# Kirkice/3DGaussian

Hardware: AMD Instinct MI355X
Metric: Mpixels/sec fwd+bwd @1M Gaussians 800×800; PSNR vs torch ref (higher is better)
Workload: dtype f32 (splat contractions on v_mfma_f32_32x32x16_f16 with f32 accumulation; every operand in two round-to-nearest f16 pieces, pre-scaled into f16's normal range, three piece products: <= 3*2^-22 per product, forward and backward; no-depth-gradient mode); 1 GPU; C4: 1000000 Gaussians, 50 orbit views 800x800, fwd+bwd+grad all-reduce+Adam per step; gaussians=1000000, views=50, width=800, height=800, tile=32, seed=0, parallelism=view-sharded dp1, gaussian_order=morton (trainer layout, re-established every 16 steps)

## Files before the change

### 3dgaussian_amd/csrc/gr_hip.hip

```cpp

#include <hip/hip_runtime.h>
#include <hipcub/hipcub.hpp>
#include <rocprim/rocprim.hpp>

#include <cmath>
#include <cstdint>
#include <cstdio>
#include <cstdlib>
#include <cstring>
#include <atomic>
#include <mutex>
#include <string>
#include <type_traits>
#include <vector>

#include "../../include/gr_hip.h"

#ifndef GR_TAIL2
#define GR_TAIL2 1
#endif
#ifndef GR_DEBUG_PREP_REPS
#define GR_DEBUG_PREP_REPS 1
#endif
#ifndef GR_DEBUG_BIN_REPS
// ... 324 lines not shown
  int* ticket;
};

struct Scratch {
  uint32_t* keys_in;
  int* ids_in;
  float* fwd_part;
  int2* pairs_in;
  int2* pairs_sorted;
  void* sort_tmp;
};

inline int64_t item_cap(int tiles, int64_t K, int ch = CH) { return (K + ch - 1) / ch + tiles; }
constexpr int UF32_FRAGS = 2 * 4 * 2 * 2 * 64;
constexpr int UF32_STRIDE = UF32_FRAGS + 64;
struct TileCfg {
  int T, ch;
  size_t part_floats, uf_frags;
};
constexpr int UF_FRAGS16 = 2 * 3 * 3 * 64;
static int64_t tune_env(const char* name);
inline int chunk_of(const gr_view* v, int base, int64_t K) {
  static const int64_t force = tune_env("GR_TUNE_CHUNK");
  int64_t c = base;
  if (v->chunk > 0) {
    c = v->chunk;
  } else if (force > 0) {
    c = force;
  } else if (K >= 0) {
    c = 512;
    while (c < base && 2 * c * 1024 <= K) c *= 2;
  }
  return (int)std::min<int64_t>(8192, std::max<int64_t>(64, (c + 63) / 64 * 64));
}
inline TileCfg tile_cfg(const gr_view* v, int64_t K = -1) {
  return tile_of(v) == T32 ? TileCfg{T32, chunk_of(v, CH32, K), (size_t)4 * TP32, (size_t)UF32_STRIDE}
                           : TileCfg{T, chunk_of(v, CH, K), (size_t)5 * TP, (size_t)UF_FRAGS16};
}

constexpr int FAN_STRIDE = 32;
__host__ __device__ inline size_t fan_offset(int tiles) { return ((size_t)tiles + 1 + FAN_STRIDE - 1) / FAN_STRIDE * FAN_STRIDE; }

size_t bins_fixed(int vtiles, int64_t K, size_t off[8], int ch = CH) {
  const int tiles = vtiles;
  const size_t kk = (size_t)(K > 0 ? K : 1);
  const size_t cap = (size_t)item_cap(tiles, K, ch);
  size_t o = 0;
  off[0] = o; o = align_up(o + (short_keys(tiles) ? 1 : kk) * sizeof(uint32_t));
  off[1] = o; o = align_up(o + kk * sizeof(int));
  off[2] = o; o = align_up(o + (size_t)tiles * sizeof(int2));
  off[3] = o; o = align_up(o + cap * sizeof(int4));
  off[4] = o; o = align_up(o + 2 * sizeof(int));
  off[5] = o; o = align_up(o + (size_t)tiles * sizeof(int));
  off[6] = o; o = align_up(o + kk * sizeof(int));
  off[7] = o; o = align_up(o + (fan_offset(tiles / 2) + 9 * FAN_STRIDE) * sizeof(int));
  return o;
}

size_t scratch_fixed(int vtiles, int64_t K, size_t off[5], int ch = CH, size_t part_floats = (size_t)5 * TP) {
  const int tiles = vtiles;
  const size_t kk = (size_t)(K > 0 ? K : 1);
  const size_t cap = (size_t)item_cap(tiles, K, ch);
  size_t o = 0;
  off[0] = o; o = align_up(o + kk * sizeof(uint32_t));
  off[1] = o; o = align_up(o + kk * sizeof(int));
  off[2] = o; o = align_up(o + cap * part_floats * sizeof(float));
  off[3] = o; o = align_up(o + (short_keys(tiles) ? 1 : kk) * sizeof(int2));
  off[4] = o; o = align_up(o + (short_keys(tiles) ? 1 : kk) * sizeof(int2));
  return o;
}


static int64_t tune_env(const char* name) {
  const char* e = std::getenv(name);
  return e ? std::atoll(e) : 0;
}
inline int tsort_waves(int tiles) {
  static const int64_t force = tune_env("GR_TUNE_PLACE_WAVES");
  const int64_t per_wave = 4ll * tiles, budget = 65536 - 512;
  const int w = 4 * per_wave <= budget ? 4 : 2 * per_wave <= budget ? 2 : 1;
  if (force == 8 && 8 * per_wave <= 81920 - 512) return 8;
  return force == 1 || force == 2 || force == 4 ? std::min<int>(w, (int)force) : w;
}

#ifndef GR_TS_SEG
#define GR_TS_SEG 24
#endif
constexpr int TS_SEG = GR_TS_SEG;

inline int col_width(int64_t K, int tiles) {
  static const int64_t force = tune_env("GR_TUNE_COL_TARGET");
  const int waves = tsort_waves(tiles);
  if (force > 0) return (int)((force + 64 * waves - 1) / (64 * waves) * (64 * waves));
  const int64_t kk = K > 0 ? K : 1;
  int64_t pw = 64ll * TS_SEG;
  auto cols_of = [&](int64_t w) { return (kk + w * waves - 1) / (w * waves); };
  while ((int64_t)tiles * cols_of(pw) > (1ll << 28) || ((int64_t)tiles * cols_of(pw) > kk / 2 && cols_of(2 * pw) >= 1024))
    pw *= 2;
  return (int)(pw * waves);
}
inline int cols_of(int64_t Kz, int cw) { return (int)((Kz + cw - 1) / cw); }

size_t tile_sort_tmp_bytes(int n, int64_t K, int tiles) {
  if (short_keys(tiles)) {
    const int st = tiles / 2;
    const size_t cells = (size_t)st * cols_of(K > 0 ? K : 1, col_width(K, st));
    (void)n;
    return 4 * align_up(cells * sizeof(int)) + 2 * align_up((size_t)st * sizeof(int));
  }
  size_t tmp = 0;
  (void)hipcub::DeviceRadixSort::SortPairs(nullptr, tmp, (const uint32_t*)nullptr, (uint32_t*)nullptr, (const int2*)nullptr,
                                           (int2*)nullptr, (int)(K > 0 ? K : 1), 0, bits_for((uint32_t)tiles),
                                           (hipStream_t)0);
  return tmp;
}

template <typename KeyT>
size_t sort_tmp_bytes(int64_t K, int bits) {
  size_t tmp = 0;
  (void)hipcub::DeviceRadixSort::SortPairs(nullptr, tmp, (KeyT*)nullptr, (KeyT*)nullptr, (int*)nullptr, (int*)nullptr,
                                     (int)(K > 0 ? K : 1), 0, bits, (hipStream_t)0);
  return tmp;
}

Bins bins_view(void* base, int tiles, int64_t K, int ch = CH) {
  size_t off[8];
  bins_fixed(tiles, K, off, ch);
  char* b = (char*)base;
  Bins r;
  r.keys = (uint32_t*)(b + off[0]);
  r.pairs = (int*)(b + off[1]);
  r.ranges = (int2*)(b + off[2]);
  r.items = (int4*)(b + off[3]);
  r.num_items = (int*)(b + off[4]);
  r.tile_item0 = (int*)(b + off[5]);
  r.pos_of = (int*)(b + off[6]);
  r.ticket = (int*)(b + off[7]);
  return r;
}

Scratch scratch_view(void* base, int tiles, int64_t K, int ch = CH, size_t part_floats = (size_t)5 * TP) {
  size_t off[5];
  const size_t fixed = scratch_fixed(tiles, K, off, ch, part_floats);
  char* b = (char*)base;
  Scratch r;
  r.keys_in = (uint32_t*)(b + off[0]);
  r.ids_in = (int*)(b + off[1]);
  r.fwd_part = (float*)(b + off[2]);
  r.pairs_in = (int2*)(b + off[3]);
  r.pairs_sorted = (int2*)(b + off[4]);
  r.sort_tmp = b + fixed;
  return r;
}

template <int NW>
__device__ __forceinline__ unsigned long long block_exclusive_scan(unsigned long long x, unsigned long long* sh,
                                                                   unsigned long long& total) {
  const int lane = (int)threadIdx.x & 63, w = (int)threadIdx.x >> 6;
  unsigned long long inc = x;
#pragma unroll
  for (int o = 1; o < 64; o <<= 1) {
    const unsigned long long y = __shfl_up(inc, o);
    if (lane >= o) inc += y;
  }
  __syncthreads();
  if (lane == 63) sh[w] = inc;
// ... 569 lines not shown
  k_tile_count_body(a.Z, a.tiles, b.block, b.grid);
}
__global__ __launch_bounds__(256) void k_tile_count(k_tile_count_args a) {
  k_tile_count_run(a, own_block());
}
__global__ __launch_bounds__(256) void k_tile_count_views(VBatch<k_tile_count_args> B) {
  const VBlock b = vbatch_block(B);
  k_tile_count_run(B.a[b.view], b);
}


#ifndef GR_CS_T
#define GR_CS_T 16
#endif
#ifndef GR_CS_THREADS
#define GR_CS_THREADS 256
#endif
#ifndef GR_CS_R
#define GR_CS_R 96
#endif
constexpr int CS_T = GR_CS_T, CS_G = GR_CS_THREADS / GR_CS_T, CS_R = GR_CS_R;

__device__ __forceinline__ void tile_colscan_block(const TZone& zz, int tiles, int bx) {
  const int cols = zz.cols;
  const int* __restrict__ M = zz.M;
  int* __restrict__ S = zz.S;
  int* __restrict__ T = zz.T;
  __shared__ int part[CS_G][CS_T + 1];
  const int tl = (int)threadIdx.x % CS_T, g = (int)threadIdx.x / CS_T;
  const int t = bx * CS_T + tl;
  const int per = (cols + CS_G - 1) / CS_G;
  const int c0 = min(cols, g * per), c1 = min(cols, c0 + per);
  const bool regs = per <= CS_R;
  int val[CS_R];
  int sum = 0;
  if (t < tiles) {
    if (regs) {
#pragma unroll
      for (int q = 0; q < CS_R; ++q) val[q] = c0 + q < c1 ? M[(size_t)(c0 + q) * tiles + t] : 0;
#pragma unroll
      for (int q = 0; q < CS_R; ++q) sum += val[q];
    } else {
#pragma unroll 8
      for (int c = c0; c < c1; ++c) sum += M[(size_t)c * tiles + t];
    }
  }
  part[g][tl] = sum;
  __syncthreads();
  if (g == 0) {
    int run = 0;
    for (int u = 0; u < CS_G; ++u) {
      const int v = part[u][tl];
      part[u][tl] = run;
      run += v;
    }
    if (t < tiles) st_through(&T[t], run);
  }
  __syncthreads();
  if (t < tiles) {
    int run = part[g][tl];
    if (regs) {
#pragma unroll
      for (int q = 0; q < CS_R; ++q)
        if (c0 + q < c1) {
          S[(size_t)(c0 + q) * tiles + t] = run;
          run += val[q];
        }
    } else {
#pragma unroll 8
      for (int c = c0; c < c1; ++c) {
        const int v = M[(size_t)c * tiles + t];
        S[(size_t)c * tiles + t] = run;
        run += v;
      }
    }
  }
}


template <bool THROUGH, int NT>
__device__ void work_items_zones(int tiles, int Kc, const int* __restrict__ Tc, const int* __restrict__ Tt,
                                 int2* __restrict__ ranges, int4* __restrict__ items, int* __restrict__ num_items,
                                 int* __restrict__ tile_item0, int* __restrict__ ticket, int ch);
__device__ __forceinline__ void k_tile_colscan_body(TZones Z, int tiles, int2* __restrict__ ranges,
                                                             int4* __restrict__ items, int* __restrict__ num_items,
                                                             int* __restrict__ tile_item0, int* __restrict__ ticket, const BI blockIdx, const BI gridDim) {
  __shared__ int last;
  const TZone zz = zone_at(Z, (int)blockIdx.y);
  if (zz.K > 0) tile_colscan_block(zz, tiles, (int)blockIdx.x);
  const int nb = (int)(gridDim.x * gridDim.y);
  if (!arrive_last_of(ticket + fan_offset(tiles), nb, (int)(blockIdx.y * gridDim.x + blockIdx.x), &last)) return;
  const TZone z0 = zone_at(Z, 0), z1 = zone_at(Z, 1);
  work_items_zones<true, GR_CS_THREADS>(tiles, z1.zbase, z0.K > 0 ? z0.T : nullptr, z1.K > 0 ? z1.T : nullptr,
                                  ranges, items, num_items, tile_item0, ticket, Z.ch);
}
struct k_tile_colscan_args {
  TZones Z;
  int tiles;
  int2* ranges;
  int4* items;
  int* num_items;
  int* tile_item0;
  int* ticket;
};
__device__ __forceinline__ void k_tile_colscan_run(const k_tile_colscan_args& a, const VBlock& b) {
  k_tile_colscan_body(a.Z, a.tiles, a.ranges, a.items, a.num_items, a.tile_item0, a.ticket, b.block, b.grid);
}
__global__ __launch_bounds__(GR_CS_THREADS) void k_tile_colscan(k_tile_colscan_args a) {
  k_tile_colscan_run(a, own_block());
}
__global__ __launch_bounds__(GR_CS_THREADS) void k_tile_colscan_views(VBatch<k_tile_colscan_args> B) {
  const VBlock b = vbatch_block(B);
  k_tile_colscan_run(B.a[b.view], b);
}



__device__ __forceinline__ void ts_load(int64_t kb, int64_t k1, int64_t klast, int lane, const uint16_t* __restrict__ keys,
                                        const int* __restrict__ ids_in, int (&d)[TS_SEG], int (&id)[TS_SEG]) {
#pragma unroll
  for (int j = 0; j < TS_SEG; ++j) {
    const int64_t k = kb + j * 64 + lane;
    const int64_t kc = k < k1 ? k : klast;
    const int key = (int)keys[kc];
    id[j] = ids_in[kc];
    d[j] = k < k1 ? key : -1;
  }
}

__device__ __forceinline__ void ts_place(int lane, int bits, int* my, const int (&d)[TS_SEG], const int (&id)[TS_SEG],
                                         int kseg, int* __restrict__ pairs_out, int* __restrict__ pos_of) {
  const uint64_t below = (1ull << lane) - 1ull;
#pragma unroll
  for (int j = 0; j < TS_SEG; ++j) {
    const bool ok = d[j] >= 0;
    const uint64_t live = __ballot(ok);
    if (live == 0) break;
    const int rel = d[j] - __builtin_amdgcn_readfirstlane(d[j]) + TS_RH;
    const bool near = __ballot(ok && (unsigned)rel >= 2u * TS_RH) == 0;
    const int key = near ? rel : d[j];
    const int nb = near && TS_RB < bits ? TS_RB : bits;
    unsigned mlo = (unsigned)live, mhi = (unsigned)(live >> 32);
    for (int b = 0; b < nb; ++b) {
      const int bm = __builtin_amdgcn_sbfe(key, b, 1);
      const uint64_t v = __ballot(bm != 0);
      mlo &= ~((unsigned)v ^ (unsigned)bm);
      mhi &= ~((unsigned)(v >> 32) ^ (unsigned)bm);
    }
    const uint64_t m = ((uint64_t)mhi << 32) | mlo;
    if (ok) {
      const int pos = my[d[j]] + __popcll(m & below);
      pairs_out[pos] = id[j];
      pos_of[kseg + j * 64 + lane] = pos;
      __builtin_amdgcn_wave_barrier();
      if ((m >> lane) == 1ull) my[d[j]] = pos + 1;
    }
  }
}

constexpr int RUNQ = 10;
template <bool THROUGH, int NT>
__device__ void work_items_zones(int tiles, int Kc, const int* __restrict__ Tc, const int* __restrict__ Tt,
                                 int2* __restrict__ ranges, int4* __restrict__ items, int* __restrict__ num_items,
                                 int* __restrict__ tile_item0, int* __restrict__ ticket, int ch) {
  __shared__ unsigned long long sh[NT / 64];
  const int per = (tiles + NT - 1) / NT;
  const int t0 = min(tiles, (int)threadIdx.x * per), t1 = min(tiles, t0 + per);
  int rc_[RUNQ], rt_[RUNQ];
  auto ld = [&](const int* T, int t) { return !T || t >= t1 ? 0 : THROUGH ? ld_through(T + t) : T[t]; };
  auto load_run = [&](int b) {
#pragma unroll
    for (int q = 0; q < RUNQ; ++q) {
      rc_[q] = ld(Tc, b + q);
      rt_[q] = ld(Tt, b + q);
    }
  };
  int sc = 0, st = 0, sch = 0, se = 0;
  for (int b = t0; b < t1; b += RUNQ) {
    load_run(b);
#pragma unroll
    for (int q = 0; q < RUNQ; ++q) {
      const int nc = rc_[q], nt = rt_[q];
      sc += nc;
      st += nt;
      const int nch = chunks_of(nc, ch) + chunks_of(nt, ch);
      sch += nch;
      se += nch == 0 && b + q < t1;
    }
  }
  unsigned long long t1v, t2v;
  const unsigned long long e1 = block_exclusive_scan<NT / 64>((unsigned long long)sc | ((unsigned long long)st << 32), sh, t1v);
  const unsigned long long e2 = block_exclusive_scan<NT / 64>((unsigned long long)sch | ((unsigned long long)se << 32), sh, t2v);
  sc = (int)(e1 & 0xffffffffull);
  st = (int)(e1 >> 32);
  sch = (int)(e2 & 0xffffffffull);
  se = (int)(e2 >> 32);
  const int total = (int)(t2v & 0xffffffffull), empties = (int)(t2v >> 32);
  se += total;
  for (int b = t0; b < t1; b += RUNQ) {
    if (t1 - t0 > RUNQ) load_run(b);
#pragma unroll
    for (int q = 0; q < RUNQ; ++q) {
      const int t = b + q;
      if (t < t1) {
        const int nc = rc_[q], nt = rt_[q];
        const int2 rc = nc > 0 ? make_int2(sc, sc + nc) : make_int2(0, 0);
        const int2 rt = nt > 0 ? make_int2(Kc + st, Kc + st + nt) : make_int2(0, 0);
        const int chc = chunks_of(nc, ch), cht = chunks_of(nt, ch);
        ranges[2 * t] = rc;
        ranges[2 * t + 1] = rt;
        tile_item0[2 * t] = sch;
        tile_item0[2 * t + 1] = sch + chc;
        ticket[t] = 0;
        for (int c = 0; c < chc; ++c) items[sch + c] = make_int4(2 * t, rc.x + c * ch, min(rc.y, rc.x + (c + 1) * ch), c);
        for (int c = 0; c < cht; ++c)
          items[sch + chc + c] = make_int4(2 * t + 1, rt.x + c * ch, min(rt.y, rt.x + (c + 1) * ch), c);
        if (chc + cht == 0) {
          tile_item0[2 * t] = tile_item0[2 * t + 1] = se;
          items[se++] = make_int4(2 * t, 0, 0, 0);
        }
        sc += nc;
        st += nt;
        sch += chc + cht;
      }
    }
  }
  if (threadIdx.x == 0) {
    num_items[0] = total + empties;
    num_items[1] = total;
  }
  if (threadIdx.x < 9) ticket[fan_offset(tiles) + FAN_STRIDE * threadIdx.x] = 0;
}

#ifndef GR_PLACE_WAVES
#define GR_PLACE_WAVES 3
#endif
constexpr int TS_CQ = 8;
template <int WAVES>
__device__ __forceinline__ void k_tile_place_body(TZones Z, int tiles, int bits,
                                                                    const int2* __restrict__ ranges,
                                                                    int* __restrict__ pairs_out, int* __restrict__ pos_of, const BI blockIdx, const BI gridDim) {
  extern __shared__ int cur[];
  constexpr int NT = 64 * WAVES;
  int c;
  const int zone = tzone_of(Z, (int)blockIdx.x, c);
  const TZone zz = zone_at(Z, zone);
  const int64_t K = zz.K;
  const int zbase = zz.zbase;
  const uint16_t* __restrict__ keys = zz.keys;
  const int* __restrict__ ids_in = zz.ids;
  const int* __restrict__ S = zz.S + (size_t)c * tiles;
  const int w = (int)threadIdx.x >> 6, lane = (int)threadIdx.x & 63;
  int* my = cur + (size_t)w * tiles;
  int64_t kc0, kc1;
  column_range(Z, K, c, kc0, kc1);
  if (kc1 <= kc0) return;
  const int64_t steps = (kc1 - kc0 + 63) / 64, wsteps = (steps + WAVES - 1) / WAVES;
  const int64_t k0 = min(kc1, kc0 + (int64_t)w * wsteps * 64), k1 = min(kc1, k0 + wsteps * 64);
  const int nseg = (int)((wsteps + TS_SEG - 1) / TS_SEG);
  int d[TS_SEG], id[TS_SEG];
  ts_load(k0, k1, K - 1, lane, keys, ids_in, d, id);
  int rx[TS_CQ], sx[TS_CQ];
  auto load_bases = [&](int t0) {
#pragma unroll
    for (int q = 0; q < TS_CQ; ++q) {
      const int t = min(t0 + q * NT, tiles - 1);
      rx[q] = ranges[2 * t + zone].x;
      sx[q] = S[t];
    }
  };
  load_bases((int)threadIdx.x);
  for (int t = lane; t < tiles; t += 64) my[t] = 0;
  __builtin_amdgcn_wave_barrier();
  for (int seg = 0; seg < nseg; ++seg) {
    if (seg > 0) ts_load(k0 + (int64_t)seg * 64 * TS_SEG, k1, K - 1, lane, keys, ids_in, d, id);
#pragma unroll
    for (int j = 0; j < TS_SEG; ++j) atomicAdd(&my[d[j] < 0 ? 0 : d[j]], (d[j] < 0 ? 0 : 1) + (id[j] >> 31));
  }
  __syncthreads();
  for (int t0 = threadIdx.x; t0 < tiles; t0 += TS_CQ * NT) {
    if (t0 != (int)threadIdx.x) load_bases(t0);
#pragma unroll
    for (int q = 0; q < TS_CQ; ++q) {
      const int t = t0 + q * NT;
      if (t >= tiles) break;
      int r = rx[q] + sx[q];
#pragma unroll
      for (int u = 0; u < WAVES; ++u) {
        const int m = cur[(size_t)u * tiles + t];
        cur[(size_t)u * tiles + t] = r;
        r += m;
      }
    }
  }
  __syncthreads();
  if (nseg == 1) {
    ts_place(lane, bits, my, d, id, zbase + (int)k0, pairs_out, pos_of);
  } else {
    for (int seg = 0; seg < nseg; ++seg) {
      ts_load(k0 + (int64_t)seg * 64 * TS_SEG, k1, K - 1, lane, keys, ids_in, d, id);
      ts_place(lane, bits, my, d, id, zbase + (int)(k0 + (int64_t)seg * 64 * TS_SEG), pairs_out, pos_of);
    }
  }
}
struct k_tile_place_args {
  TZones Z;
  int tiles;
  int bits;
  const int2* ranges;
  int* pairs_out;
  int* pos_of;
};
template <int WAVES>
__device__ __forceinline__ void k_tile_place_run(const k_tile_place_args& a, const VBlock& b) {
  k_tile_place_body<WAVES>(a.Z, a.tiles, a.bits, a.ranges, a.pairs_out, a.pos_of, b.block, b.grid);
}
template <int WAVES>
__global__ __launch_bounds__(64 * WAVES, GR_PLACE_WAVES) void k_tile_place(k_tile_place_args a) {
  k_tile_place_run<WAVES>(a, own_block());
}
template <int WAVES>
__global__ __launch_bounds__(64 * WAVES, GR_PLACE_WAVES) void k_tile_place_views(VBatch<k_tile_place_args> B) {
  const VBlock b = vbatch_block(B);
  k_tile_place_run<WAVES>(B.a[b.view], b);
}


__device__ __forceinline__ void split3(float x, float& hi, float& mid, float& lo) {
  hi = __uint_as_float(__float_as_uint(x) & 0xffff0000u);
  const float r1 = x - hi;
  mid = __uint_as_float(__float_as_uint(r1) & 0xffff0000u);
  lo = r1 - mid;
}
__device__ __forceinline__ unsigned pack_bf16(float a, float b) {
  return __builtin_amdgcn_perm(__float_as_uint(b), __float_as_uint(a), 0x07060302u);
}

typedef short s16x8 __attribute__((ext_vector_type(8)));
typedef float f32x16 __attribute__((ext_vector_type(16)));

__device__ __forceinline__ s16x8 as_frag(uint4 u) {
  s16x8 f;
  __builtin_memcpy(&f, &u, sizeof(f));
  return f;
}

__device__ __forceinline__ void split3_frag(const float (&v)[8], s16x8 (&f)[3]) {
  float hi[8], mid[8], lo[8];
#pragma unroll
  for (int j = 0; j < 8; ++j) split3(v[j], hi[j], mid[j], lo[j]);
  f[0] = as_frag(make_uint4(pack_bf16(hi[0], hi[1]), pack_bf16(hi[2], hi[3]), pack_bf16(hi[4], hi[5]), pack_bf16(hi[6], hi[7])));
  f[1] = as_frag(make_uint4(pack_bf16(mid[0], mid[1]), pack_bf16(mid[2], mid[3]), pack_bf16(mid[4], mid[5]),
                            pack_bf16(mid[6], mid[7])));
  f[2] = as_frag(make_uint4(pack_bf16(lo[0], lo[1]), pack_bf16(lo[2], lo[3]), pack_bf16(lo[4], lo[5]), pack_bf16(lo[6], lo[7])));
}
typedef __bf16 bf16x2_t __attribute__((ext_vector_type(2)));
typedef float f32x2_t __attribute__((ext_vector_type(2)));
__device__ __forceinline__ void split2_frag(const float (&v)[8], s16x8 (&f)[2]) {
  unsigned h[4], l[4];
#pragma unroll
  for (int p = 0; p < 4; ++p) {
    const f32x2_t x = {v[2 * p], v[2 * p + 1]};
    const bf16x2_t hb = __builtin_convertvector(x, bf16x2_t);
    __builtin_memcpy(&h[p], &hb, 4);
    const f32x2_t r = {x.x - __uint_as_float(h[p] << 16), x.y - __uint_as_float(h[p] & 0xffff0000u)};
    const bf16x2_t lb = __builtin_convertvector(r, bf16x2_t);
    __builtin_memcpy(&l[p], &lb, 4);
  }
  f[0] = as_frag(make_uint4(h[0], h[1], h[2], h[3]));
  f[1] = as_frag(make_uint4(l[0], l[1], l[2], l[3]));
}
__device__ __forceinline__ f32x4 mfma16(const s16x8& a, const s16x8& b, f32x4 c) {
  return __builtin_amdgcn_mfma_f32_16x16x32_bf16(a, b, c, 0, 0, 0);
}
__device__ __forceinline__ f32x4 mfma16_split3(const s16x8 (&a)[3], const s16x8 (&b)[3], f32x4 c) {
  c = mfma16(a[2], b[0], c);
  c = mfma16(a[1], b[1], c);
  c = mfma16(a[0], b[2], c);
  c = mfma16(a[1], b[0], c);
  c = mfma16(a[0], b[1], c);
  return mfma16(a[0], b[0], c);
}
template <bool B3>
__device__ __forceinline__ f32x4 mfma16_split2(const s16x8 (&a)[2], const s16x8 (&b)[3], f32x4 c) {
  c = mfma16(a[1], b[0], c);
  if constexpr (B3) c = mfma16(a[0], b[2], c);
  c = mfma16(a[0], b[1], c);
  return mfma16(a[0], b[0], c);
}

__device__ __forceinline__ void split2_frag2(const f32x2_t (&v)[4], s16x8 (&f)[2]) {
  float u[8];
#pragma unroll
  for (int p = 0; p < 4; ++p) {
    u[2 * p] = v[p].x;
    u[2 * p + 1] = v[p].y;
  }
  split2_frag(u, f);
}

__device__ __forceinline__ void split3_frag2(const f32x2_t (&v)[4], s16x8 (&f)[3]) {
  float u[8];
#pragma unroll
  for (int p = 0; p < 4; ++p) {
    u[2 * p] = v[p].x;
    u[2 * p + 1] = v[p].y;
  }
// ... 3797 lines not shown
  char* q = (char*)c.sc.sort_tmp;
  for (int z = 0; z < 2; ++z) {
    TZone& zz = Z.z[z];
    zz.K = Kr[z];
    zz.cols = cols_of(Kr[z], Z.cw);
    zz.zbase = z == 0 ? 0 : (int)Kc;
    zz.keys = (const uint16_t*)c.sc.keys_in + (z == 0 ? 0 : Kc);
    zz.ids = c.sc.ids_in + (z == 0 ? 0 : Kc);
    zz.M = (int*)q;
    q += align_up(cells * sizeof(int));
    zz.S = (int*)q;
    q += align_up(cells * sizeof(int));
    zz.T = (int*)q;
    q += align_up((size_t)c.tiles * sizeof(int));
  }
  return Z;
}

struct ParamsIn {
  const float *means = nullptr, *scales = nullptr, *colors = nullptr;
  int color_dim = 3;
  const float* opacities = nullptr;
};
struct GradsOut {
  float *d_means = nullptr, *d_scales = nullptr, *d_colors = nullptr, *d_opacities = nullptr;
  int accumulate = 0;
};
struct ViewLoss {
  const float *t_rgb = nullptr, *t_mask = nullptr;
  float w_sil = 0.0f;
  const float* t_depth = nullptr;
  float w_depth = 0.0f, g_scale = 0.0f;
  float* loss_out = nullptr;
  bool ssim_entry = false;
  float w_dssim = 0.0f;
  bool expo_entry = false;
  const float* exposure = nullptr;
  float* d_exposure = nullptr;
  bool wgt_entry = false;
  const float* t_weight = nullptr;
};
struct BwdRequest {
  const gr_view* view = nullptr;
  int n = 0;
  const gr_plan* plan = nullptr;
  const void *geom = nullptr, *bins = nullptr;
  const float* saved = nullptr;
  void* ws = nullptr;
  size_t ws_bytes = 0;
  void* stream = nullptr;
  ParamsIn params;
  const float *g_rgb = nullptr, *g_alpha = nullptr, *g_depth = nullptr;
  ViewLoss loss;
  GradsOut grads;
  float *sums = nullptr, *sums3 = nullptr;
  const int* sum_index = nullptr;
};

static L1Args fit_l1_args(const ViewCtx& c, const ViewLoss& vl) {
  L1Args l1{vl.t_rgb, vl.t_mask, vl.w_sil, vl.g_scale, nullptr};
  if (!vl.t_rgb) return l1;
  l1.tile_loss = c.w.tile_loss;
  l1.loss_out = vl.loss_out;
  l1.n1 = (int64_t)(3 * c.HW);
  l1.n2 = (int64_t)(vl.t_mask ? c.HW : 0);
  if (vl.t_depth) {
    l1.t_depth = vl.t_depth;
    l1.w_depth = vl.w_depth;
    l1.dscal = c.w.dscal;
  }
  return l1;
}

static k_emit_offsets_args emit_offsets_args(const ViewCtx& c) {
  return {c.vk, c.n, (const int4*)c.g.rect, (const Cnt2*)c.g.counts, (const unsigned long long*)c.g.total,
          (Cnt2*)c.g.offsets, (const float4*)c.g.rec, (uint16_t*)c.sc.keys_in, c.sc.ids_in,
          c.b.ticket + fan_offset(c.tiles)};
}
static k_tile_count_args tile_count_args(const ViewCtx& c, const TZones& Z) { return {Z, c.tiles}; }
static k_tile_colscan_args tile_colscan_args(const ViewCtx& c, const TZones& Z) {
  return {Z, c.tiles, c.b.ranges, c.b.items, c.b.num_items, c.b.tile_item0, c.b.ticket};
}
static k_tile_place_args tile_place_args(const ViewCtx& c, const TZones& Z) {
  return {Z, c.tiles, bits_for((uint32_t)c.tiles), (const int2*)c.b.ranges, c.b.pairs, c.b.pos_of};
}
static k_raster_fwd_mfma_args fwd_mfma_args(const ViewCtx& c, float* out_rgb, float* out_alpha, float* out_depth,
                                            float* saved, const L1Args& l1, uint4* UF) {
  return {c.vk, c.n, (const int4*)c.b.items, (const int*)c.b.num_items, (const int2*)c.b.ranges, (const int*)c.b.pairs,
          (const float4*)c.g.rec, c.sc.fwd_part, out_rgb, out_alpha, out_depth, (float4*)saved,
          saved ? saved + 4 * c.HW : nullptr, l1, UF, (const int*)(c.n > 0 && c.K() > 0 ? c.g.f16_sa : nullptr),
          (const int*)c.b.tile_item0, c.b.ticket, c.tc.ch};
}
static k_fwd32_l1_args fwd32_args(const ViewCtx& c, float* out_rgb, float* out_alpha, const L1Args& l1, uint4* UF) {
  return {c.vk, c.n, (const int4*)c.b.items, (const int*)c.b.num_items, (const int2*)c.b.ranges, (const int*)c.b.pairs,
          (const float4*)c.g.rec, c.sc.fwd_part, out_rgb, out_alpha, l1, UF,
          (const int*)(c.n > 0 && c.K() > 0 ? c.g.f16_sa : nullptr), (const int*)c.b.tile_item0, c.b.ticket, c.tc.ch};
}
static k_raster_bwd_bf16_args bwd_bf16_args(const ViewCtx& c, float* depth3) {
  return {c.vk, c.n, (const int4*)c.b.items, (const int*)c.b.num_items, (const int*)c.b.pairs, (const float4*)c.g.rec,
          (const uint4*)c.w.UF, c.w.partials, depth3};
}
static k_bwd32_args bwd32_args(const ViewCtx& c) {
  return {c.vk, c.n, (const int4*)c.b.items, (const int*)c.b.num_items, (const int*)c.b.pairs, (const float4*)c.g.rec,
          (const uint4*)c.w.UF, c.w.partials};
}
static k_depth_tile_max_args depth_tile_max_args(const ViewCtx& c, const float* saved) {
  return {c.vk, (const float4*)saved, saved + 4 * c.HW, c.w.tile_aux, c.w.dscal, c.b.ticket};
}
static k_depth_tile_sums_args depth_tile_sums_args(const ViewCtx& c, const float* saved, const float* t_depth,
                                                   float w_depth, float g_scale) {
  return {c.vk, (const float4*)saved, saved + 4 * c.HW, t_depth, c.w.dscal, c.w.tile_loss, c.w.tile_aux, (int64_t)c.HW,
          w_depth, g_scale, c.b.ticket};
}
static k_pixel_grads_args pixel_grads_args(const ViewCtx& c, const float* saved, const float* g_rgb, const float* g_alpha,
                                           const float* g_depth, int pieces, const L1Args& l1, bool depth) {
  return {c.vk, (const float4*)saved, saved + 4 * c.HW, g_rgb, g_alpha, g_depth, c.w.UF, pieces, l1, depth, c.b.ticket};
}
static k_gather_view_args gather_args(const ViewCtx& c, float* sums, float* sums3, bool depth) {
  return {c.n, (const Cnt2*)c.g.offsets, (const int*)c.b.pos_of, (const float4*)c.w.partials, (float2*)sums,
          depth ? (const float*)c.depth3() : nullptr, depth ? sums3 : nullptr};
}
struct TilePlace {
  void (*one)(k_tile_place_args);
  void (*views)(VBatch<k_tile_place_args>);
  int threads;
  size_t lds;
};
static TilePlace tile_place_of(int tiles) {
  const int waves = tsort_waves(tiles);
  const size_t lds = (size_t)tiles * sizeof(int) * waves;
  if (waves == 8) return {k_tile_place<8>, k_tile_place_views<8>, 512, lds};
  if (waves == 4) return {k_tile_place<4>, k_tile_place_views<4>, 256, lds};
  if (waves == 2) return {k_tile_place<2>, k_tile_place_views<2>, 128, lds};
  return {k_tile_place<1>, k_tile_place_views<1>, 64, lds};
}

template <class A>
static void launch_one(void (*kern)(A), dim3 grid, int threads, size_t lds, hipStream_t s, const A& a) {
  hipLaunchKernelGGL(kern, grid, dim3(threads), lds, s, a);
}
template <class A>
static void vb_add(VBatch<A>& B, const A& a, int blocks, int gx = 0) {
  B.a[B.nv] = a;
  B.gx[B.nv] = gx > 0 ? gx : (blocks > 0 ? blocks : 1);
  B.first[B.nv + 1] = B.first[B.nv] + (blocks > 0 ? blocks : 0);
  ++B.nv;
}
template <class A>
static VBatch<A> vb_new() {
  static_assert(sizeof(VBatch<A>) <= 4096, "batched kernel arguments exceed 4 KiB");
  VBatch<A> B;
  B.nv = 0;
  B.first[0] = 0;
  return B;
}
#define GR_VB_LAUNCH(kern, B, threads, lds, s)                                                   \
  do {                                                                                           \
    if ((B).first[(B).nv] > 0) {                                                                 \
      hipLaunchKernelGGL(kern, dim3((unsigned)(B).first[(B).nv]), dim3(threads), lds, s, (B));   \
      GR_HIP_TRY(hipGetLastError());                                                             \
    }                                                                                            \
  } while (0)

static gr_status bin_impl(const ViewCtx& c, hipStream_t s) {
  const gr_view* v = c.view;
  const int n = c.n, tiles = c.tiles, vtiles = 2 * tiles;
  const int64_t num_pairs = c.K();
  const Bins& b = c.b;
  const Scratch& sc = c.sc;
  prof_mark(PROF_BINNING, s);
  if (n > 0 && num_pairs > 0) {
    const Geom& g = c.g;
    if (short_keys(vtiles)) {
      const TZones Z = tile_zones(c);
      launch_one(k_emit_offsets, dim3(blocks_for(n)), 256, 0, s, emit_offsets_args(c));
      GR_HIP_TRY(hipGetLastError());
      const int blocks = Z.z[0].cols + Z.z[1].cols;
      launch_one(k_tile_count, dim3(blocks), 256, (size_t)tiles * sizeof(int), s, tile_count_args(c, Z));
      GR_HIP_TRY(hipGetLastError());
      launch_one(k_tile_colscan, dim3((tiles + CS_T - 1) / CS_T, 2), CS_T * CS_G, 0, s, tile_colscan_args(c, Z));
      GR_HIP_TRY(hipGetLastError());
      const TilePlace place = tile_place_of(tiles);
      launch_one(place.one, dim3(blocks), place.threads, place.lds, s, tile_place_args(c, Z));
      GR_HIP_TRY(hipGetLastError());
    } else {
      if (v->device_counts)
        return set_error(GR_ERR_INVALID_ARGUMENT, "device_counts views need the counting-sort binning (<= 8,192 tiles)");
      hipLaunchKernelGGL(k_offsets, dim3(blocks_for(n)), dim3(256), 0, s, n, (const unsigned long long*)g.counts,
                         (const unsigned long long*)g.total, g.offsets);
      GR_HIP_TRY(hipGetLastError());
      hipLaunchKernelGGL((k_emit_zones<uint32_t, true>), dim3(blocks_for(n)), dim3(256), 0, s, c.vk, n,
                         (const int4*)g.rect, (const Cnt2*)g.counts, (const Cnt2*)g.offsets, (const float4*)g.rec, sc.keys_in, sc.ids_in);
      GR_HIP_TRY(hipGetLastError());
      hipLaunchKernelGGL(k_pair_values, dim3(blocks_for(num_pairs)), dim3(256), 0, s, num_pairs, (const int*)sc.ids_in,
                         sc.pairs_in);
      GR_HIP_TRY(hipGetLastError());
      GR_HIP_TRY(hipMemsetAsync(b.ranges, 0, sizeof(int2) * vtiles, s));
      const int bits = bits_for((uint32_t)vtiles);
      size_t tmp = tile_sort_tmp_bytes(n, num_pairs, vtiles);
      GR_HIP_TRY(hipcub::DeviceRadixSort::SortPairs(sc.sort_tmp, tmp, sc.keys_in, b.keys, sc.pairs_in, sc.pairs_sorted,
                                                    (int)num_pairs, 0, bits, s));
      hipLaunchKernelGGL(k_ranges<uint32_t>, dim3(blocks_for(num_pairs)), dim3(256), 0, s, num_pairs, b.keys, b.ranges);
      GR_HIP_TRY(hipGetLastError());
      hipLaunchKernelGGL(k_pos_of, dim3(blocks_for(num_pairs)), dim3(256), 0, s, num_pairs, (const int2*)sc.pairs_sorted,
                         b.pairs, b.pos_of);
      GR_HIP_TRY(hipGetLastError());
      hipLaunchKernelGGL(k_work_items, dim3(1), dim3(WI_THREADS), 0, s, vtiles, (const int2*)b.ranges, b.items, b.num_items,
                         b.tile_item0, b.ticket, c.tc.ch);
    }
  } else {
    if (n > 0) GR_HIP_TRY(hipMemsetAsync(c.g.offsets, 0, (size_t)n * sizeof(unsigned long long), s));
    GR_HIP_TRY(hipMemsetAsync(b.ranges, 0, sizeof(int2) * vtiles, s));
    hipLaunchKernelGGL(k_work_items, dim3(1), dim3(WI_THREADS), 0, s, vtiles, (const int2*)b.ranges, b.items, b.num_items,
                       b.tile_item0, b.ticket, c.tc.ch);
  }
  GR_HIP_TRY(hipGetLastError());
  prof_mark(PROF_BINNING, s);
  return GR_OK;
}

static gr_status fwd_impl(const gr_view* v, int n, const gr_plan* plan, const void* geom, void* bins, size_t bins_bytes,
                          void* scratch, size_t scratch_bytes, float* out_rgb, float* out_alpha, float* out_depth,
                          float* saved, void* stream, const ViewLoss* l1, void* ws, size_t ws_bytes,
                          bool depth_sums = false) {
  gr_status st = check_view(v);
  if (st != GR_OK) return st;
  if (!plan) return set_error(GR_ERR_INVALID_ARGUMENT, "plan is null");
  if (plan->num_pairs < 0 || plan->num_slots < 0) return set_error(GR_ERR_OVERFLOW, "pair count overflows int32");
  if (!l1 && !saved) return set_error(GR_ERR_INVALID_ARGUMENT, "saved is required");
  if (l1 && (!ws || ws_bytes < gr_bwd_bytes(v, n, plan) || !l1->loss_out))
    return set_error(GR_ERR_WORKSPACE, "gr_fwd_render_l1: backward workspace too small (or null loss)");
  if (n > 0 && (!geom || !bins)) return set_error(GR_ERR_INVALID_ARGUMENT, "null workspace");
  if (bins_bytes < gr_bins_bytes(v, n, plan)) return set_error(GR_ERR_WORKSPACE, "bins workspace too small");
  if (scratch_bytes < gr_fwd_scratch_bytes(v, n, plan) || !scratch)
    return set_error(GR_ERR_WORKSPACE, "forward scratch workspace too small");
  hipStream_t s = (hipStream_t)stream;
  const ViewCtx c = view_ctx(v, n, plan, geom, bins, scratch, l1 ? ws : nullptr);
  if (v->rows > 0 && !l1)
    return set_error(GR_ERR_INVALID_ARGUMENT, "a band of tile rows (gr_view.rows): gr_fwd_render_l1 only (the fit loss)");
  if (c.tc.T == T32 && (!l1 || v->no_depth_grad != 1))
    return set_error(GR_ERR_INVALID_ARGUMENT, "32-pixel tiles (gr_view.tile = 32): gr_fwd_render_l1 with no_depth_grad = 1 only");
  if (c.tc.T == T32 && c.vk.core != c.vk.cutoff)
    return set_error(GR_ERR_INVALID_ARGUMENT, "32-pixel tiles (gr_view.tile = 32): one-zone footprint only (core_cutoff <= 0 or >= cutoff)");
  if (!v->binned) {
    for (int rep = 0; rep < GR_DEBUG_BIN_REPS; ++rep) {
      st = bin_impl(c, s);
      if (st != GR_OK) return st;
    }
  }
  L1Args la = fit_l1_args(c, l1 ? *l1 : ViewLoss{});
  if (l1) la.pieces = v->no_depth_grad == 1 ? 2 : 3;
  uint4* UF = l1 ? c.w.UF : nullptr;
  if (!(GR_DEBUG_SKIP & 1)) {
    prof_mark(PROF_RASTER_FWD, s);
    const bool f32g = v->no_depth_grad != 1;
    if (c.tc.T == T32) {
      const k_fwd32_l1_args a = fwd32_args(c, out_rgb, out_alpha, la, UF);
      hipLaunchKernelGGL(k_fwd32_l1, dim3((unsigned)c.cap), dim3(256), 0, s, a.v, a.n, a.items, a.num_items, a.ranges,
                         a.pairs, a.rec, a.fwd_part, a.out_rgb, a.out_alpha, a.l1, a.UF, a.f16_sa, a.tile_item0, a.ticket,
                         a.ch);
    } else
      launch_one(l1 ? (f32g ? k_raster_fwd_mfma<5> : k_raster_fwd_mfma<4>)
                    : (f32g ? k_raster_fwd_mfma<1>
                            : (out_depth || depth_sums ? k_raster_fwd_mfma<2> : k_raster_fwd_mfma<3>)),
                 dim3((unsigned)c.cap), 256, 0, s, fwd_mfma_args(c, out_rgb, out_alpha, out_depth, saved, la, UF));
    GR_HIP_TRY(hipGetLastError());
// ... 342 lines not shown
  r.loss.exposure = exposure;
  r.loss.d_exposure = d_exposure;
  r.sums = sums;
  r.sums3 = sums3;
  return bwd_impl(r);
}

gr_status gr_bwd_fit_weighted_gather(const gr_view* v, int n, const gr_plan* plan, const void* geom, const void* bins,
                                     const float* saved, const float* target_rgb, const float* target_mask, float w_sil,
                                     const float* target_depth, float w_depth, float g_scale, const float* target_weight,
                                     float* loss_out, void* ws, size_t ws_bytes, float* sums, float* sums3,
                                     void* stream) {
  if (!target_rgb) return set_error(GR_ERR_INVALID_ARGUMENT, "gr_bwd_fit_weighted_gather: target_rgb is null");
  if (!sums) return set_error(GR_ERR_INVALID_ARGUMENT, "gr_bwd_fit_weighted_gather: sums is null");
  if (!target_weight) return set_error(GR_ERR_INVALID_ARGUMENT, "gr_bwd_fit_weighted_gather: target_weight is null");
  BwdRequest r{v, n, plan, geom, bins, saved, ws, ws_bytes, stream};
  r.loss = {target_rgb, target_mask, w_sil, target_depth, w_depth, g_scale, loss_out};
  r.loss.wgt_entry = true;
  r.loss.t_weight = target_weight;
  r.sums = sums;
  r.sums3 = sums3;
  return bwd_impl(r);
}

gr_status gr_bwd_l1(const gr_view* v, int n, const gr_plan* plan, const float* means, const float* scales,
                    const float* colors, int color_dim, const float* opacities, const void* geom, const void* bins,
                    const float* saved, const float* target_rgb, const float* target_mask, float w_sil, float g_scale,
                    float* loss_out, float* d_means, float* d_scales, float* d_colors, float* d_opacities,
                    int accumulate, void* ws, size_t ws_bytes, void* stream) {
  if (!target_rgb) return set_error(GR_ERR_INVALID_ARGUMENT, "gr_bwd_l1: target_rgb is null");
  BwdRequest r{v, n, plan, geom, bins, saved, ws, ws_bytes, stream};
  r.params = {means, scales, colors, color_dim, opacities};
  r.loss.t_rgb = target_rgb;
  r.loss.t_mask = target_mask;
  r.loss.w_sil = w_sil;
  r.loss.g_scale = g_scale;
  r.loss.loss_out = loss_out;
  r.grads = {d_means, d_scales, d_colors, d_opacities, accumulate};
  return bwd_impl(r);
}

gr_status gr_fit_views_batched(int num_views, const gr_batch_view* bv, int n, float w_sil, float w_depth,
                                          float g_scale, void* stream) {
  if (num_views < 1 || num_views > GR_BATCH_MAX_VIEWS || !bv)
    return set_error(GR_ERR_INVALID_ARGUMENT, "gr_fit_views_batched: num_views must be in [1, GR_BATCH_MAX_VIEWS]");
  if (n <= 0) return set_error(GR_ERR_INVALID_ARGUMENT, "gr_fit_views_batched: n must be > 0");
  static_assert(GR_BATCH_MAX_VIEWS == GR_BATCH_MAX, "gr_hip.h GR_BATCH_MAX_VIEWS");
  const gr_view& v0 = bv[0].view;
  const bool depth = bv[0].target_depth != nullptr;
  for (int j = 0; j < num_views; ++j) {
    const gr_batch_view& b = bv[j];
    gr_status st = check_view(&b.view);
    if (st != GR_OK) return st;
    if (b.view.width != v0.width || b.view.height != v0.height || tile_of(&b.view) != tile_of(&v0) ||
        b.view.no_depth_grad != v0.no_depth_grad || b.view.cutoff != v0.cutoff || b.view.core_cutoff != v0.core_cutoff ||
        b.view.device_counts != v0.device_counts || (b.target_depth != nullptr) != depth)
      return set_error(GR_ERR_INVALID_ARGUMENT, "gr_fit_views_batched: the views differ in size, tile, footprint or mode");
    if (b.plan.num_pairs <= 0 || b.plan.num_slots < b.plan.num_pairs)
      return set_error(GR_ERR_INVALID_ARGUMENT, "gr_fit_views_batched: every view needs pairs (or capacities)");
    if (!b.geom || !b.bins || !b.scratch || !b.ws || !b.target_rgb || !b.sums || !b.loss || (depth && (!b.saved || !b.sums3)))
      return set_error(GR_ERR_INVALID_ARGUMENT, "gr_fit_views_batched: null pointer");
    if (b.bins_bytes < gr_bins_bytes(&b.view, n, &b.plan) || b.scratch_bytes < gr_fwd_scratch_bytes(&b.view, n, &b.plan) ||
        b.ws_bytes < gr_bwd_bytes(&b.view, n, &b.plan))
      return set_error(GR_ERR_WORKSPACE, "gr_fit_views_batched: a workspace is too small");
  }
  if (!short_keys(vtiles_of(&v0)))
    return set_error(GR_ERR_INVALID_ARGUMENT, "gr_fit_views_batched: more than 8,192 screen tiles");
  if (depth ? v0.no_depth_grad != 0 : v0.no_depth_grad != 1)
    return set_error(GR_ERR_INVALID_ARGUMENT, "gr_fit_views_batched: depth loss needs no_depth_grad = 0, the L1 path 1");
  if (depth && tile_of(&v0) != T)
    return set_error(GR_ERR_INVALID_ARGUMENT, "gr_fit_views_batched: the depth-loss path runs at 16-pixel tiles");
  for (int j = 0; j < num_views && depth; ++j)
    if (bv[j].view.rows > 0)
      return set_error(GR_ERR_INVALID_ARGUMENT, "gr_fit_views_batched: a band of tile rows needs the L1 path (no depth loss)");
  hipStream_t s = (hipStream_t)stream;
  const int tiles = vtiles_of(&v0) / 2;
  ViewCtx ctx[GR_BATCH_MAX];
  for (int j = 0; j < num_views; ++j)
    ctx[j] = view_ctx(&bv[j].view, n, &bv[j].plan, bv[j].geom, bv[j].bins, bv[j].scratch, bv[j].ws);
  auto Be = vb_new<k_emit_offsets_args>();
  auto Bc = vb_new<k_tile_count_args>();
  auto Bs = vb_new<k_tile_colscan_args>();
  auto Bp = vb_new<k_tile_place_args>();
  for (int j = 0; j < num_views; ++j) {
    const ViewCtx& c = ctx[j];
    const TZones Z = tile_zones(c);
    const int cols = Z.z[0].cols + Z.z[1].cols;
    vb_add(Be, emit_offsets_args(c), blocks_for(n));
    vb_add(Bc, tile_count_args(c, Z), cols);
    const int gxs = (tiles + CS_T - 1) / CS_T;
    vb_add(Bs, tile_colscan_args(c, Z), 2 * gxs, gxs);
    vb_add(Bp, tile_place_args(c, Z), cols);
  }
  GR_VB_LAUNCH(k_emit_offsets_views, Be, 256, 0, s);
  GR_VB_LAUNCH(k_tile_count_views, Bc, 256, (size_t)tiles * sizeof(int), s);
  GR_VB_LAUNCH(k_tile_colscan_views, Bs, CS_T * CS_G, 0, s);
  const TilePlace place = tile_place_of(tiles);
  GR_VB_LAUNCH(place.views, Bp, place.threads, place.lds, s);

  auto Bg = vb_new<k_gather_view_args>();
  if (!depth) {
    auto Bf = vb_new<k_fwd32_l1_args>();
    auto Bf16 = vb_new<k_raster_fwd_mfma_args>();
    auto Bb = vb_new<k_bwd32_args>();
    auto Bb16 = vb_new<k_raster_bwd_bf16_args>();
    for (int j = 0; j < num_views; ++j) {
      const gr_batch_view& b = bv[j];
      const ViewCtx& c = ctx[j];
      L1Args la = fit_l1_args(c, {b.target_rgb, b.target_mask, w_sil, b.target_depth, w_depth, g_scale, b.loss});
      la.pieces = 2;
      const int cap = (int)c.cap;
      if (c.tc.T == T32) {
        vb_add(Bf, fwd32_args(c, nullptr, nullptr, la, c.w.UF), cap);
        vb_add(Bb, bwd32_args(c), cap);
      } else {
        vb_add(Bf16, fwd_mfma_args(c, nullptr, nullptr, nullptr, nullptr, la, c.w.UF), cap);
        vb_add(Bb16, bwd_bf16_args(c, nullptr), cap);
      }
      vb_add(Bg, gather_args(c, b.sums, nullptr, false), (n + 63) / 64);
    }
    GR_VB_LAUNCH(k_fwd32_l1_views, Bf, 256, 0, s);
    GR_VB_LAUNCH(k_raster_fwd_mfma_views<4>, Bf16, 256, 0, s);
    GR_VB_LAUNCH(k_bwd32_views, Bb, 256, 0, s);
    GR_VB_LAUNCH((k_raster_bwd_bf16_views<false, 2>), Bb16, 256, 0, s);
    GR_VB_LAUNCH(k_gather_view_views<false>, Bg, 256, 0, s);
    return GR_OK;
  }
  auto Bf = vb_new<k_raster_fwd_mfma_args>();
  auto Bm = vb_new<k_depth_tile_max_args>();
  auto Bd = vb_new<k_depth_tile_sums_args>();
  auto Bu = vb_new<k_pixel_grads_args>();
  auto Bb = vb_new<k_raster_bwd_bf16_args>();
  for (int j = 0; j < num_views; ++j) {
    const gr_batch_view& b = bv[j];
    const ViewCtx& c = ctx[j];
    const int cap = (int)c.cap;
    vb_add(Bf, fwd_mfma_args(c, nullptr, nullptr, nullptr, b.saved, fit_l1_args(c, ViewLoss{}), nullptr), cap);
    vb_add(Bm, depth_tile_max_args(c, b.saved), tiles);
    vb_add(Bd, depth_tile_sums_args(c, b.saved, b.target_depth, w_depth, g_scale), tiles);
    const L1Args l1 = fit_l1_args(c, {b.target_rgb, b.target_mask, w_sil, b.target_depth, w_depth, g_scale, b.loss});
    vb_add(Bu, pixel_grads_args(c, b.saved, nullptr, nullptr, nullptr, 3, l1, true), tiles);
    vb_add(Bb, bwd_bf16_args(c, c.depth3()), cap);
    vb_add(Bg, gather_args(c, b.sums, b.sums3, true), (n + 63) / 64);
  }
  GR_VB_LAUNCH(k_raster_fwd_mfma_views<1>, Bf, 256, 0, s);
  GR_VB_LAUNCH(k_depth_tile_max_views, Bm, 256, 0, s);
  GR_VB_LAUNCH(k_depth_tile_sums_views, Bd, 256, 0, s);
  GR_VB_LAUNCH(k_pixel_grads_views, Bu, 256, 0, s);
  GR_VB_LAUNCH((k_raster_bwd_bf16_views<true, 3>), Bb, 256, 0, s);
  GR_VB_LAUNCH(k_gather_view_views<true>, Bg, 256, 0, s);
  return GR_OK;
}

gr_status gr_bwd_splat(const gr_view* v, int n, const gr_plan* plan, const void* geom, const void* bins, void* ws,
                       size_t ws_bytes, void* stream) {
  gr_status st = check_view(v);
  if (st != GR_OK) return st;
  if (!v->no_depth_grad)
    return set_error(GR_ERR_INVALID_ARGUMENT, "gr_bwd_splat: the view must have no_depth_grad = 1 or 2");
  if (!plan) return set_error(GR_ERR_INVALID_ARGUMENT, "plan is null");
  if (plan->num_pairs < 0) return set_error(GR_ERR_OVERFLOW, "pair count overflows int32");
  if (n <= 0 || plan->num_pairs == 0) return GR_OK;
  if (!geom || !bins) return set_error(GR_ERR_INVALID_ARGUMENT, "null pointer");
  if (!ws || ws_bytes < gr_bwd_bytes(v, n, plan)) return set_error(GR_ERR_WORKSPACE, "backward workspace too small");
  hipStream_t s = (hipStream_t)stream;
  const ViewCtx c = view_ctx(v, n, plan, geom, bins, nullptr, ws);
  if (c.tc.T == T32 && v->no_depth_grad != 1)
    return set_error(GR_ERR_INVALID_ARGUMENT, "32-pixel tiles (gr_view.tile = 32): no_depth_grad = 1 only");
  if (GR_DEBUG_SKIP & 2) return GR_OK;
  prof_mark(PROF_RASTER_BWD, s);
  if (c.tc.T == T32) {
    const k_bwd32_args a = bwd32_args(c);
    hipLaunchKernelGGL(k_bwd32, dim3((unsigned)c.cap), dim3(256), 0, s, a.v, a.n, a.items, a.num_items, a.pairs, a.rec,
                       a.UF, a.partials);
  } else
    launch_one(v->no_depth_grad == 1 ? k_raster_bwd_bf16<false, 2> : k_raster_bwd_bf16<false, 3>, dim3((unsigned)c.cap),
               256, 0, s, bwd_bf16_args(c, nullptr));
  GR_HIP_TRY(hipGetLastError());
  prof_mark(PROF_RASTER_BWD, s);
  return GR_OK;
// ... 645 lines not shown
```

Baseline: 1526 Mpixels/sec.

## Move work-item construction from colscan tail into an extra tile-place block for small grids

```diff
diff --git a/3dgaussian_amd/csrc/gr_hip.hip b/3dgaussian_amd/csrc/gr_hip.hip
--- a/3dgaussian_amd/csrc/gr_hip.hip
+++ b/3dgaussian_amd/csrc/gr_hip.hip
@@ -430,6 +430,9 @@
   if (force == 8 && 8 * per_wave <= 81920 - 512) return 8;
   return force == 1 || force == 2 || force == 4 ? std::min<int>(w, (int)force) : w;
 }
+
+constexpr int TS_SQ = 4, TS_SMALL_TILES = 256 * TS_SQ;
+inline bool tsort_small(int tiles) { return tiles <= TS_SMALL_TILES && tsort_waves(tiles) == 4; }
 
 #ifndef GR_TS_SEG
 #define GR_TS_SEG 24
@@ -1165,12 +1168,14 @@
 __device__ void work_items_zones(int tiles, int Kc, const int* __restrict__ Tc, const int* __restrict__ Tt,
                                  int2* __restrict__ ranges, int4* __restrict__ items, int* __restrict__ num_items,
                                  int* __restrict__ tile_item0, int* __restrict__ ticket, int ch);
+template <bool TAIL>
 __device__ __forceinline__ void k_tile_colscan_body(TZones Z, int tiles, int2* __restrict__ ranges,
                                                              int4* __restrict__ items, int* __restrict__ num_items,
                                                              int* __restrict__ tile_item0, int* __restrict__ ticket, const BI blockIdx, const BI gridDim) {
   __shared__ int last;
   const TZone zz = zone_at(Z, (int)blockIdx.y);
   if (zz.K > 0) tile_colscan_block(zz, tiles, (int)blockIdx.x);
+  if (!TAIL) return;
   const int nb = (int)(gridDim.x * gridDim.y);
   if (!arrive_last_of(ticket + fan_offset(tiles), nb, (int)(blockIdx.y * gridDim.x + blockIdx.x), &last)) return;
   const TZone z0 = zone_at(Z, 0), z1 = zone_at(Z, 1);
@@ -1186,15 +1191,18 @@
   int* tile_item0;
   int* ticket;
 };
+template <bool TAIL>
 __device__ __forceinline__ void k_tile_colscan_run(const k_tile_colscan_args& a, const VBlock& b) {
-  k_tile_colscan_body(a.Z, a.tiles, a.ranges, a.items, a.num_items, a.tile_item0, a.ticket, b.block, b.grid);
-}
+  k_tile_colscan_body<TAIL>(a.Z, a.tiles, a.ranges, a.items, a.num_items, a.tile_item0, a.ticket, b.block, b.grid);
+}
+template <bool TAIL>
 __global__ __launch_bounds__(GR_CS_THREADS) void k_tile_colscan(k_tile_colscan_args a) {
-  k_tile_colscan_run(a, own_block());
-}
+  k_tile_colscan_run<TAIL>(a, own_block());
+}
+template <bool TAIL>
 __global__ __launch_bounds__(GR_CS_THREADS) void k_tile_colscan_views(VBatch<k_tile_colscan_args> B) {
   const VBlock b = vbatch_block(B);
-  k_tile_colscan_run(B.a[b.view], b);
+  k_tile_colscan_run<TAIL>(B.a[b.view], b);
 }
 
 
@@ -1319,14 +1327,28 @@
 #define GR_PLACE_WAVES 3
 #endif
 constexpr int TS_CQ = 8;
-template <int WAVES>
+struct TileLists {
+  int2* ranges;
+  int4* items;
+  int* num_items;
+  int* tile_item0;
+  int* ticket;
+};
+template <int WAVES, bool SMALL>
 __device__ __forceinline__ void k_tile_place_body(TZones Z, int tiles, int bits,
                                                                     const int2* __restrict__ ranges,
-                                                                    int* __restrict__ pairs_out, int* __restrict__ pos_of, const BI blockIdx, const BI gridDim) {
+                                                                    int* __restrict__ pairs_out, int* __restrict__ pos_of,
+                                                                    const TileLists& wl, const BI blockIdx, const BI gridDim) {
   extern __shared__ int cur[];
   constexpr int NT = 64 * WAVES;
+  if (SMALL && blockIdx.x == 0) {
+    const TZone z0 = zone_at(Z, 0), z1 = zone_at(Z, 1);
+    work_items_zones<false, NT>(tiles, z1.zbase, z0.K > 0 ? z0.T : nullptr, z1.K > 0 ? z1.T : nullptr, wl.ranges, wl.items,
+                                wl.num_items, wl.tile_item0, wl.ticket, Z.ch);
+    return;
+  }
   int c;
-  const int zone = tzone_of(Z, (int)blockIdx.x, c);
+  const int zone = tzone_of(Z, (int)blockIdx.x - (SMALL ? 1 : 0), c);
   const TZone zz = zone_at(Z, zone);
   const int64_t K = zz.K;
   const int zbase = zz.zbase;
@@ -1341,6 +1363,11 @@
   const int64_t steps = (kc1 - kc0 + 63) / 64, wsteps = (steps + WAVES - 1) / WAVES;
   const int64_t k0 = min(kc1, kc0 + (int64_t)w * wsteps * 64), k1 = min(kc1, k0 + wsteps * 64);
   const int nseg = (int)((wsteps + TS_SEG - 1) / TS_SEG);
+  int tv[TS_SQ];
+  if (SMALL) {
+#pragma unroll
+    for (int q = 0; q < TS_SQ; ++q) tv[q] = (int)threadIdx.x * TS_SQ + q < tiles ? zz.T[(int)threadIdx.x * TS_SQ + q] : 0;
+  }
   int d[TS_SEG], id[TS_SEG];
   ts_load(k0, k1, K - 1, lane, keys, ids_in, d, id);
   int rx[TS_CQ], sx[TS_CQ];
@@ -1348,11 +1375,25 @@
 #pragma unroll
     for (int q = 0; q < TS_CQ; ++q) {
       const int t = min(t0 + q * NT, tiles - 1);
-      rx[q] = ranges[2 * t + zone].x;
+      if (!SMALL) rx[q] = ranges[2 * t + zone].x;
       sx[q] = S[t];
     }
   };
   load_bases((int)threadIdx.x);
+  int* tstart = cur + (size_t)WAVES * tiles;
+  if (SMALL) {
+    __shared__ unsigned long long sh[WAVES];
+    int sum = 0;
+#pragma unroll
+    for (int q = 0; q < TS_SQ; ++q) sum += tv[q];
+    unsigned long long all;
+    int run = zbase + (int)block_exclusive_scan<WAVES>((unsigned long long)sum, sh, all);
+#pragma unroll
+    for (int q = 0; q < TS_SQ; ++q) {
+      if ((int)threadIdx.x * TS_SQ + q < tiles) tstart[(int)threadIdx.x * TS_SQ + q] = run;
+      run += tv[q];
+    }
+  }
   for (int t = lane; t < tiles; t += 64) my[t] = 0;
   __builtin_amdgcn_wave_barrier();
   for (int seg = 0; seg < nseg; ++seg) {
@@ -1367,7 +1408,7 @@
     for (int q = 0; q < TS_CQ; ++q) {
       const int t = t0 + q * NT;
       if (t >= tiles) break;
-      int r = rx[q] + sx[q];
+      int r = (SMALL ? tstart[t] : rx[q]) + sx[q];
 #pragma unroll
       for (int u = 0; u < WAVES; ++u) {
         const int m = cur[(size_t)u * tiles + t];
@@ -1393,19 +1434,20 @@
   const int2* ranges;
   int* pairs_out;
   int* pos_of;
+  TileLists w;
 };
-template <int WAVES>
+template <int WAVES, bool SMALL>
 __device__ __forceinline__ void k_tile_place_run(const k_tile_place_args& a, const VBlock& b) {
-  k_tile_place_body<WAVES>(a.Z, a.tiles, a.bits, a.ranges, a.pairs_out, a.pos_of, b.block, b.grid);
-}
-template <int WAVES>
+  k_tile_place_body<WAVES, SMALL>(a.Z, a.tiles, a.bits, a.ranges, a.pairs_out, a.pos_of, a.w, b.block, b.grid);
+}
+template <int WAVES, bool SMALL = false>
 __global__ __launch_bounds__(64 * WAVES, GR_PLACE_WAVES) void k_tile_place(k_tile_place_args a) {
-  k_tile_place_run<WAVES>(a, own_block());
-}
-template <int WAVES>
+  k_tile_place_run<WAVES, SMALL>(a, own_block());
+}
+template <int WAVES, bool SMALL = false>
 __global__ __launch_bounds__(64 * WAVES, GR_PLACE_WAVES) void k_tile_place_views(VBatch<k_tile_place_args> B) {
   const VBlock b = vbatch_block(B);
-  k_tile_place_run<WAVES>(B.a[b.view], b);
+  k_tile_place_run<WAVES, SMALL>(B.a[b.view], b);
 }
 
 
@@ -5369,7 +5411,8 @@
   return {Z, c.tiles, c.b.ranges, c.b.items, c.b.num_items, c.b.tile_item0, c.b.ticket};
 }
 static k_tile_place_args tile_place_args(const ViewCtx& c, const TZones& Z) {
-  return {Z, c.tiles, bits_for((uint32_t)c.tiles), (const int2*)c.b.ranges, c.b.pairs, c.b.pos_of};
+  return {Z, c.tiles, bits_for((uint32_t)c.tiles), (const int2*)c.b.ranges, c.b.pairs, c.b.pos_of,
+          {c.b.ranges, c.b.items, c.b.num_items, c.b.tile_item0, c.b.ticket}};
 }
 static k_raster_fwd_mfma_args fwd_mfma_args(const ViewCtx& c, float* out_rgb, float* out_alpha, float* out_depth,
                                             float* saved, const L1Args& l1, uint4* UF) {
@@ -5412,15 +5455,26 @@
   void (*views)(VBatch<k_tile_place_args>);
   int threads;
   size_t lds;
+  int extra;
 };
 static TilePlace tile_place_of(int tiles) {
   const int waves = tsort_waves(tiles);
   const size_t lds = (size_t)tiles * sizeof(int) * waves;
-  if (waves == 8) return {k_tile_place<8>, k_tile_place_views<8>, 512, lds};
-  if (waves == 4) return {k_tile_place<4>, k_tile_place_views<4>, 256, lds};
-  if (waves == 2) return {k_tile_place<2>, k_tile_place_views<2>, 128, lds};
-  return {k_tile_place<1>, k_tile_place_views<1>, 64, lds};
-}
+  if (tsort_small(tiles)) return {k_tile_place<4, true>, k_tile_place_views<4, true>, 256, lds + (size_t)tiles * sizeof(int), 1};
+  if (waves == 8) return {k_tile_place<8>, k_tile_place_views<8>, 512, lds, 0};
+  if (waves == 4) return {k_tile_place<4>, k_tile_place_views<4>, 256, lds, 0};
+  if (waves == 2) return {k_tile_place<2>, k_tile_place_views<2>, 128, lds, 0};
+  return {k_tile_place<1>, k_tile_place_views<1>, 64, lds, 0};
+}
+struct TileColscan {
+  void (*one)(k_tile_colscan_args);
+  void (*views)(VBatch<k_tile_colscan_args>);
+};
+static TileColscan tile_colscan_of(int tiles) {
+  if (tsort_small(tiles)) return {k_tile_colscan<false>, k_tile_colscan_views<false>};
+  return {k_tile_colscan<true>, k_tile_colscan_views<true>};
+}
+static dim3 tile_colscan_grid(const TZones& Z, int tiles) { return dim3((tiles + CS_T - 1) / CS_T, Z.z[1].cols > 0 ? 2 : 1); }
 
 template <class A>
 static void launch_one(void (*kern)(A), dim3 grid, int threads, size_t lds, hipStream_t s, const A& a) {
@@ -5465,10 +5519,10 @@
       const int blocks = Z.z[0].cols + Z.z[1].cols;
       launch_one(k_tile_count, dim3(blocks), 256, (size_t)tiles * sizeof(int), s, tile_count_args(c, Z));
       GR_HIP_TRY(hipGetLastError());
-      launch_one(k_tile_colscan, dim3((tiles + CS_T - 1) / CS_T, 2), CS_T * CS_G, 0, s, tile_colscan_args(c, Z));
+      launch_one(tile_colscan_of(tiles).one, tile_colscan_grid(Z, tiles), CS_T * CS_G, 0, s, tile_colscan_args(c, Z));
       GR_HIP_TRY(hipGetLastError());
       const TilePlace place = tile_place_of(tiles);
-      launch_one(place.one, dim3(blocks), place.threads, place.lds, s, tile_place_args(c, Z));
+      launch_one(place.one, dim3(blocks + place.extra), place.threads, place.lds, s, tile_place_args(c, Z));
       GR_HIP_TRY(hipGetLastError());
     } else {
       if (v->device_counts)
@@ -5977,20 +6031,20 @@
   auto Bc = vb_new<k_tile_count_args>();
   auto Bs = vb_new<k_tile_colscan_args>();
   auto Bp = vb_new<k_tile_place_args>();
+  const TilePlace place = tile_place_of(tiles);
   for (int j = 0; j < num_views; ++j) {
     const ViewCtx& c = ctx[j];
     const TZones Z = tile_zones(c);
     const int cols = Z.z[0].cols + Z.z[1].cols;
     vb_add(Be, emit_offsets_args(c), blocks_for(n));
     vb_add(Bc, tile_count_args(c, Z), cols);
-    const int gxs = (tiles + CS_T - 1) / CS_T;
-    vb_add(Bs, tile_colscan_args(c, Z), 2 * gxs, gxs);
-    vb_add(Bp, tile_place_args(c, Z), cols);
+    const dim3 gs = tile_colscan_grid(Z, tiles);
+    vb_add(Bs, tile_colscan_args(c, Z), (int)(gs.x * gs.y), (int)gs.x);
+    vb_add(Bp, tile_place_args(c, Z), cols + place.extra);
   }
   GR_VB_LAUNCH(k_emit_offsets_views, Be, 256, 0, s);
   GR_VB_LAUNCH(k_tile_count_views, Bc, 256, (size_t)tiles * sizeof(int), s);
-  GR_VB_LAUNCH(k_tile_colscan_views, Bs, CS_T * CS_G, 0, s);
-  const TilePlace place = tile_place_of(tiles);
+  GR_VB_LAUNCH(tile_colscan_of(tiles).views, Bs, CS_T * CS_G, 0, s);
   GR_VB_LAUNCH(place.views, Bp, place.threads, place.lds, s);
 
   auto Bg = vb_new<k_gather_view_args>();
```

Result: no change. 1530 Mpixels/sec (median of 5 runs) (+0.3%).
